# ShardianLabs/EphemeralNet

Measured on AMD Instinct MI355X. Metric: GiB/s ChaCha20-Poly1305 seal+open (device-resident) at 1/2/4/8 MI355X, higher is better.
Workload: dtype u32; 1 GPU; C2: 65536 x 4096 B records, per-record (key, nonce), AEAD seal+open, device-resident; records_per_gpu=65536, record_bytes=4096, lanes_per_record=2, parallelism=records split over 1 GPU(s), no collective

## Files before the change

### ephemeralnet_amd/build.py

```python
from __future__ import annotations

import hashlib
import json
import os
import platform
import re
import subprocess
import sys
import time
from concurrent.futures import ThreadPoolExecutor

PKG = os.path.dirname(os.path.abspath(__file__))
ROOT = os.path.dirname(PKG)
CSRC = os.path.join(PKG, "csrc")
LIB = os.path.join(PKG, "libenet_crypto.so")
OBJ = os.path.join(PKG, "build")
LIB_TOOLS = os.path.join(PKG, "libenet_crypto_tools.so")
OBJ_TOOLS = os.path.join(PKG, "build_tools")
SOURCES = ["records.hip", "segments.hip", "stream.hip", "sha.hip", "pow.hip", "duplex.hip", "duplex_split.hip",
           "chunk_frames.hip", "announce_frames.hip", "control_frames.hip",
           "shamir.hip", "shamir_host.cpp", "handshake.hip",
           "capi.cpp", "long_records.cpp", "chunk_hybrid.cpp", "staging.cpp", "scalar_api.cpp", "batch_records.cpp",
           "batch_staged.cpp", "pipeline.cpp", "host_engine.cpp",
           "frame_queue.cpp", "queue_core.cpp", "host_batch.cpp", "host_topo.cpp"]
HEADERS = ["enet_device.hpp", "enet_internal.hpp", "long_route.hpp", "record_route.hpp", "long_records.hpp", "records_body.hpp",
           "stream_common.hpp", "stream_map.hpp", "duplex_common.hpp", "pow_common.hpp", "host_engine.hpp", "scalar.hpp", "staging.hpp", "api_common.hpp", "host_batch.hpp", "host_topo.hpp", "gf256.hpp",
           "queue_knobs.hpp", "wire_host.hpp", "queue_slots.hpp", "queue_core.hpp"]
HIPCC = os.environ.get("HIPCC", "/opt/rocm/bin/hipcc")
CFLAGS = ["--offload-arch=gfx950", "-O3", "-std=c++20", "-fPIC",
          "-fvisibility=hidden", "-Wall", "-Wno-unused-function",
          "-I" + os.path.join(ROOT, "include")]
LDFLAGS = ["--offload-arch=gfx950", "-fPIC", "-shared"]


DEVICE_HEADERS = ["enet_device.hpp", "enet_internal.hpp", "long_route.hpp", "record_route.hpp", "records_body.hpp", "stream_common.hpp",
                  "stream_map.hpp", "duplex_common.hpp", "pow_common.hpp", "chacha_lockstep_asm.hpp", "gf256.hpp"]


def _headers(src: str = "") -> list[str]:
    if src.endswith(".hip"):
        return [os.path.join(CSRC, f) for f in DEVICE_HEADERS if os.path.exists(os.path.join(CSRC, f))]
    deps = [os.path.join(CSRC, f) for f in HEADERS + ["chacha_lockstep_asm.hpp"]]
    for dp, _, fs in os.walk(os.path.join(ROOT, "include")):
        deps += [os.path.join(dp, f) for f in fs]
    return [d for d in deps if os.path.exists(d)]


def _obj(src: str, obj_dir: str = OBJ) -> str:
    return os.path.join(obj_dir, os.path.splitext(src)[0] + ".o")


def _reads_tools_macro(src: str) -> bool:
    todo, seen = [src], set()
    while todo:
        f = todo.pop()
        if f in seen:
            continue
        seen.add(f)
        try:
            with open(os.path.join(CSRC, f)) as fh:
                text = fh.read()
        except OSError:
            continue
        if "ENET_TOOLS_BUILD" in text:
            return True
        todo += re.findall(r'^\s*#\s*include\s*"([^"]+)"', text, re.M)
    return False


# ... 91 lines not shown
```

### ephemeralnet_amd/csrc/chacha_lockstep_asm.hpp

```cpp
#pragma once

#define ENET_LS_C0 \
    "v_add_u32_e32 %0, %0, %4\n" \
    "v_add_u32_e32 %1, %1, %5\n" \
    "v_add_u32_e32 %2, %2, %6\n" \
    "v_add_u32_e32 %3, %3, %7\n" \
    "v_add_u32_e32 %16, %16, %20\n" \
    "v_add_u32_e32 %17, %17, %21\n" \
    "v_add_u32_e32 %18, %18, %22\n" \
    "v_add_u32_e32 %19, %19, %23\n" \
    "v_xor_b32_e32 %12, %12, %0\n" \
    "v_xor_b32_e32 %13, %13, %1\n" \
    "v_xor_b32_e32 %14, %14, %2\n" \
    "v_xor_b32_e32 %15, %15, %3\n" \
    "v_xor_b32_e32 %28, %28, %16\n" \
    "v_xor_b32_e32 %29, %29, %17\n" \
    "v_xor_b32_e32 %30, %30, %18\n" \
    "v_xor_b32_e32 %31, %31, %19\n" \
    "v_alignbit_b32 %12, %12, %12, 16\n" \
    "v_alignbit_b32 %13, %13, %13, 16\n" \
    "v_alignbit_b32 %14, %14, %14, 16\n" \
    "v_alignbit_b32 %15, %15, %15, 16\n" \
    "v_alignbit_b32 %28, %28, %28, 16\n" \
    "v_alignbit_b32 %29, %29, %29, 16\n" \
// ... 370 lines not shown
    "v_alignbit_b32 %22, %22, %22, 25\n" \
    "v_alignbit_b32 %23, %23, %23, 25\n" \
    "v_alignbit_b32 %20, %20, %20, 25\n" \
    "s_barrier\n"

#define ENET_LS_D3_NB \
    "v_add_u32_e32 %10, %10, %15\n" \
    "v_add_u32_e32 %11, %11, %12\n" \
    "v_add_u32_e32 %8, %8, %13\n" \
    "v_add_u32_e32 %9, %9, %14\n" \
    "v_add_u32_e32 %26, %26, %31\n" \
    "v_add_u32_e32 %27, %27, %28\n" \
    "v_add_u32_e32 %24, %24, %29\n" \
    "v_add_u32_e32 %25, %25, %30\n" \
    "v_xor_b32_e32 %5, %5, %10\n" \
    "v_xor_b32_e32 %6, %6, %11\n" \
    "v_xor_b32_e32 %7, %7, %8\n" \
    "v_xor_b32_e32 %4, %4, %9\n" \
    "v_xor_b32_e32 %21, %21, %26\n" \
    "v_xor_b32_e32 %22, %22, %27\n" \
    "v_xor_b32_e32 %23, %23, %24\n" \
    "v_xor_b32_e32 %20, %20, %25\n" \
    "v_alignbit_b32 %5, %5, %5, 25\n" \
    "v_alignbit_b32 %6, %6, %6, 25\n" \
    "v_alignbit_b32 %7, %7, %7, 25\n" \
    "v_alignbit_b32 %4, %4, %4, 25\n" \
    "v_alignbit_b32 %21, %21, %21, 25\n" \
    "v_alignbit_b32 %22, %22, %22, 25\n" \
    "v_alignbit_b32 %23, %23, %23, 25\n" \
    "v_alignbit_b32 %20, %20, %20, 25\n"

#define ENET_LS_X32(x)                                                                    \
    : "+v"(x[0]), "+v"(x[1]), "+v"(x[2]), "+v"(x[3]), "+v"(x[4]), "+v"(x[5]), "+v"(x[6]), "+v"(x[7]), "+v"(x[8]), "+v"(x[9]), "+v"(x[10]), "+v"(x[11]), "+v"(x[12]), "+v"(x[13]), "+v"(x[14]), "+v"(x[15]), "+v"(x[16]), "+v"(x[17]), "+v"(x[18]), "+v"(x[19]), "+v"(x[20]), "+v"(x[21]), "+v"(x[22]), "+v"(x[23]), "+v"(x[24]), "+v"(x[25]), "+v"(x[26]), "+v"(x[27]), "+v"(x[28]), "+v"(x[29]), "+v"(x[30]), "+v"(x[31])
```

### ephemeralnet_amd/csrc/enet_device.hpp

```cpp
#pragma once

#include <hip/hip_runtime.h>
#include <stdint.h>

#include <type_traits>
#include <utility>

#include "chacha_lockstep_asm.hpp"

namespace enet {

constexpr uint32_t kSigma0 = 0x61707865u, kSigma1 = 0x3320646eu, kSigma2 = 0x79622d32u,
                   kSigma3 = 0x6b206574u;

__device__ __forceinline__ uint32_t rotl(uint32_t v, int s) { return __builtin_rotateleft32(v, s); }

#define ENET_QR(a, b, c, d)                  \
    do {                                     \
        a += b; d ^= a; d = rotl(d, 16);     \
        c += d; b ^= c; b = rotl(b, 12);     \
        a += b; d ^= a; d = rotl(d, 8);      \
        c += d; b ^= c; b = rotl(b, 7);      \
    } while (0)

struct ChachaRecord {
    uint32_t k[8];
    uint32_t n[3];
    uint32_t pre[12];
};

__device__ __forceinline__ void chacha_record_init(ChachaRecord& R, const uint32_t k[8],
                                                   const uint32_t n[3]) {
#pragma unroll
    for (int i = 0; i < 8; ++i) R.k[i] = k[i];
#pragma unroll
    for (int i = 0; i < 3; ++i) R.n[i] = n[i];
    uint32_t a1 = kSigma1, b1 = k[1], c1 = k[5], d1 = n[0];
    uint32_t a2 = kSigma2, b2 = k[2], c2 = k[6], d2 = n[1];
    uint32_t a3 = kSigma3, b3 = k[3], c3 = k[7], d3 = n[2];
    ENET_QR(a1, b1, c1, d1);
    ENET_QR(a2, b2, c2, d2);
    ENET_QR(a3, b3, c3, d3);
    R.pre[0] = a1; R.pre[1] = b1; R.pre[2] = c1; R.pre[3] = d1;
    R.pre[4] = a2; R.pre[5] = b2; R.pre[6] = c2; R.pre[7] = d2;
    R.pre[8] = a3; R.pre[9] = b3; R.pre[10] = c3; R.pre[11] = d3;
}

__device__ __forceinline__ void chacha_block(const ChachaRecord& R, uint32_t counter,
                                             uint32_t x[16]) {
    uint32_t x0 = kSigma0, x4 = R.k[0], x8 = R.k[4], x12 = counter;
    ENET_QR(x0, x4, x8, x12);
    uint32_t x1 = R.pre[0], x5 = R.pre[1], x9 = R.pre[2], x13 = R.pre[3];
    uint32_t x2 = R.pre[4], x6 = R.pre[5], x10 = R.pre[6], x14 = R.pre[7];
    uint32_t x3 = R.pre[8], x7 = R.pre[9], x11 = R.pre[10], x15 = R.pre[11];
    ENET_QR(x0, x5, x10, x15);
    ENET_QR(x1, x6, x11, x12);
    ENET_QR(x2, x7, x8, x13);
    ENET_QR(x3, x4, x9, x14);
#pragma unroll
    for (int i = 1; i < 10; ++i) {
        ENET_QR(x0, x4, x8, x12);
        ENET_QR(x1, x5, x9, x13);
        ENET_QR(x2, x6, x10, x14);
        ENET_QR(x3, x7, x11, x15);
        ENET_QR(x0, x5, x10, x15);
        ENET_QR(x1, x6, x11, x12);
        ENET_QR(x2, x7, x8, x13);
        ENET_QR(x3, x4, x9, x14);
    }
    x[0] = x0 + kSigma0; x[1] = x1 + kSigma1; x[2] = x2 + kSigma2; x[3] = x3 + kSigma3;
    x[4] = x4 + R.k[0]; x[5] = x5 + R.k[1]; x[6] = x6 + R.k[2]; x[7] = x7 + R.k[3];
    x[8] = x8 + R.k[4]; x[9] = x9 + R.k[5]; x[10] = x10 + R.k[6]; x[11] = x11 + R.k[7];
    x[12] = x12 + counter; x[13] = x13 + R.n[0]; x[14] = x14 + R.n[1]; x[15] = x15 + R.n[2];
}

__device__ __forceinline__ void chacha_block2(const ChachaRecord& R, uint32_t ca, uint32_t cb,
                                              uint32_t xa[16], uint32_t xb[16]) {
    uint32_t a0 = kSigma0, a4 = R.k[0], a8 = R.k[4], a12 = ca;
// ... 78 lines not shown
    auto after = [&](auto k) {
        asm volatile("" ::: "memory");
        sh(std::integral_constant<int, BASE + decltype(k)::value>{});
        asm volatile("" ::: "memory");
    };
    constexpr bool b0 = BAR == 1, b1 = BAR == 1 || BAR == 2, b2 = BAR == 1, b3 = BAR != 0;
#define ENET_LS_STEP(NAME, B)                               \
    do {                                                    \
        if constexpr (B) asm volatile(NAME ENET_LS_X32(x)); \
        else asm volatile(NAME##_NB ENET_LS_X32(x));        \
    } while (0)
    if constexpr (DIAG) {
        ENET_LS_STEP(ENET_LS_D0, b0);
        after(std::integral_constant<int, 0>{});
        ENET_LS_STEP(ENET_LS_D1, b1);
        after(std::integral_constant<int, 1>{});
        ENET_LS_STEP(ENET_LS_D2, b2);
        after(std::integral_constant<int, 2>{});
        ENET_LS_STEP(ENET_LS_D3, b3);
        after(std::integral_constant<int, 3>{});
    } else {
        ENET_LS_STEP(ENET_LS_C0, b0);
        after(std::integral_constant<int, 0>{});
        ENET_LS_STEP(ENET_LS_C1, b1);
        after(std::integral_constant<int, 1>{});
        ENET_LS_STEP(ENET_LS_C2, b2);
        after(std::integral_constant<int, 2>{});
        ENET_LS_STEP(ENET_LS_C3, b3);
        after(std::integral_constant<int, 3>{});
    }
#undef ENET_LS_STEP
}

__device__ __forceinline__ void chacha_block2_lockstep(const ChachaRecord& R, uint32_t ca, uint32_t cb,
                                                       uint32_t xa[16], uint32_t xb[16]) {
    uint32_t a0 = kSigma0, a4 = R.k[0], a8 = R.k[4], a12 = ca;
    uint32_t b0 = kSigma0, b4 = R.k[0], b8 = R.k[4], b12 = cb;
    ENET_QR(a0, a4, a8, a12);
    ENET_QR(b0, b4, b8, b12);
    uint32_t x[32];
    x[0] = a0; x[4] = a4; x[8] = a8; x[12] = a12;
    x[16] = b0; x[20] = b4; x[24] = b8; x[28] = b12;
#pragma unroll
    for (int c = 1; c < 4; ++c) {
#pragma unroll
        for (int r = 0; r < 4; ++r) {
            x[c + 4 * r] = R.pre[4 * (c - 1) + r];
            x[16 + c + 4 * r] = R.pre[4 * (c - 1) + r];
        }
    }
    chacha_half_lockstep2<true>(x);
#pragma unroll
    for (int i = 1; i < 10; ++i) {
        chacha_half_lockstep2<false>(x);
        chacha_half_lockstep2<true>(x);
    }
    const uint32_t ff[16] = {kSigma0, kSigma1, kSigma2, kSigma3, R.k[0], R.k[1], R.k[2], R.k[3],
                             R.k[4], R.k[5], R.k[6], R.k[7], 0u, R.n[0], R.n[1], R.n[2]};
#pragma unroll
    for (int i = 0; i < 16; ++i) {
        xa[i] = x[i] + (i == 12 ? ca : ff[i]);
        xb[i] = x[16 + i] + (i == 12 ? cb : ff[i]);
    }
}

constexpr uint32_t M26 = 0x3ffffffu;
// ... 50 lines not shown
    uint32_t h0 = hin[0], h1 = hin[1], h2 = hin[2], h3 = hin[3], h4 = hin[4], c;
#pragma unroll
    for (int pass = 0; pass < 2; ++pass) {
        c = h0 >> 26; h0 &= M26; h1 += c;
        c = h1 >> 26; h1 &= M26; h2 += c;
        c = h2 >> 26; h2 &= M26; h3 += c;
        c = h3 >> 26; h3 &= M26; h4 += c;
        c = h4 >> 26; h4 &= M26; h0 += c * 5u;
    }
    c = h0 >> 26; h0 &= M26; h1 += c;
    uint32_t g0 = h0 + 5u; c = g0 >> 26; g0 &= M26;
    uint32_t g1 = h1 + c; c = g1 >> 26; g1 &= M26;
    uint32_t g2 = h2 + c; c = g2 >> 26; g2 &= M26;
    uint32_t g3 = h3 + c; c = g3 >> 26; g3 &= M26;
    uint32_t g4 = h4 + c - (1u << 26);
    const uint32_t use_g = (g4 >> 31) - 1u;
    h0 = (h0 & ~use_g) | (g0 & use_g);
    h1 = (h1 & ~use_g) | (g1 & use_g);
    h2 = (h2 & ~use_g) | (g2 & use_g);
    h3 = (h3 & ~use_g) | (g3 & use_g);
    h4 = (h4 & ~use_g) | (g4 & use_g);
    uint64_t f;
    f = (uint64_t)(h0 | (h1 << 26)) + s[0]; tag[0] = (uint32_t)f;
    f = (uint64_t)((h1 >> 6) | (h2 << 20)) + s[1] + (f >> 32); tag[1] = (uint32_t)f;
    f = (uint64_t)((h2 >> 12) | (h3 << 14)) + s[2] + (f >> 32); tag[2] = (uint32_t)f;
    f = (uint64_t)((h3 >> 18) | (h4 << 8)) + s[3] + (f >> 32); tag[3] = (uint32_t)f;
}

__device__ __forceinline__ void pclamp(uint32_t r[5], uint32_t w0, uint32_t w1, uint32_t w2,
                                       uint32_t w3) {
    plimbs(r, w0 & 0x0fffffffu, w1 & 0x0ffffffcu, w2 & 0x0ffffffcu, w3 & 0x0ffffffcu);
}

struct PolyR32 {
    uint32_t r0, r1, r2, r3, s1, s2, s3;
};

__device__ __forceinline__ PolyR32 polyr32_make(uint32_t w0, uint32_t w1, uint32_t w2, uint32_t w3) {
    PolyR32 R;
    R.r0 = w0 & 0x0fffffffu;
    R.r1 = w1 & 0x0ffffffcu;
    R.r2 = w2 & 0x0ffffffcu;
    R.r3 = w3 & 0x0ffffffcu;
    R.s1 = R.r1 + (R.r1 >> 2);
    R.s2 = R.r2 + (R.r2 >> 2);
    R.s3 = R.r3 + (R.r3 >> 2);
    return R;
}

__device__ __forceinline__ void poly32_block(uint32_t h[5], const PolyR32& R, uint32_t m0,
                                             uint32_t m1, uint32_t m2, uint32_t m3,
                                             uint32_t hibit) {
    unsigned cy;
    const uint32_t a0 = __builtin_addc(h[0], m0, 0u, &cy);
    const uint32_t a1 = __builtin_addc(h[1], m1, cy, &cy);
    const uint32_t a2 = __builtin_addc(h[2], m2, cy, &cy);
    const uint32_t a3 = __builtin_addc(h[3], m3, cy, &cy);
    const uint32_t a4 = h[4] + hibit + cy;
    const uint64_t d0 = (uint64_t)a0 * R.r0 + (uint64_t)a1 * R.s3 + (uint64_t)a2 * R.s2 +
                        (uint64_t)a3 * R.s1;
    const uint64_t e1 = (uint64_t)a0 * R.r1 + (uint64_t)a1 * R.r0 + (uint64_t)a2 * R.s3 +
                        (uint64_t)a3 * R.s2 + (uint64_t)a4 * R.s1;
    const uint64_t e2 = (uint64_t)a0 * R.r2 + (uint64_t)a1 * R.r1 + (uint64_t)a2 * R.r0 +
                        (uint64_t)a3 * R.s3 + (uint64_t)a4 * R.s2;
    const uint64_t e3 = (uint64_t)a0 * R.r3 + (uint64_t)a1 * R.r2 + (uint64_t)a2 * R.r1 +
                        (uint64_t)a3 * R.r0 + (uint64_t)a4 * R.s3;
    const uint32_t x0 = (uint32_t)d0;
    const uint32_t x1 = __builtin_addc((uint32_t)e1, (uint32_t)(d0 >> 32), 0u, &cy);
    const uint32_t c1 = (uint32_t)(e1 >> 32) + cy;
    const uint32_t x2 = __builtin_addc((uint32_t)e2, c1, 0u, &cy);
    const uint32_t c2 = (uint32_t)(e2 >> 32) + cy;
    const uint32_t x3 = __builtin_addc((uint32_t)e3, c2, 0u, &cy);
    const uint32_t c3 = (uint32_t)(e3 >> 32) + cy;
    const uint32_t t4 = a4 * R.r0 + c3;
    const uint32_t f = (t4 >> 2) * 5u;
    h[0] = __builtin_addc(x0, f, 0u, &cy);
    h[1] = __builtin_addc(x1, 0u, cy, &cy);
    h[2] = __builtin_addc(x2, 0u, cy, &cy);
    h[3] = __builtin_addc(x3, 0u, cy, &cy);
    h[4] = (t4 & 3u) + cy;
}

__device__ __forceinline__ void h32_to_limbs(const uint32_t h[5], uint32_t l[5]) {
    l[0] = h[0] & M26;
    l[1] = __builtin_amdgcn_alignbit(h[1], h[0], 26) & M26;
    l[2] = __builtin_amdgcn_alignbit(h[2], h[1], 20) & M26;
    l[3] = __builtin_amdgcn_alignbit(h[3], h[2], 14) & M26;
    l[4] = (h[3] >> 8) | (h[4] << 24);
}

__device__ __forceinline__ void ppow(const uint32_t r[5], uint32_t e, uint32_t x[5]) {
#pragma unroll
    for (int i = 0; i < 5; ++i) x[i] = r[i];
    const Pmul mr = pmul_make(r);
    const int top = 31 - __builtin_clz(e);
    for (int b = top - 1; b >= 0; --b) {
        pmul(x, pmul_make(x));
        if ((e >> b) & 1u) pmul(x, mr);
    }
}

__device__ __forceinline__ uint32_t bswap32(uint32_t v) { return __builtin_bswap32(v); }
__device__ __forceinline__ uint32_t rotr(uint32_t v, int s) { return __builtin_rotateright32(v, s); }

__constant__ static const uint32_t kSha256K[64] = {
    0x428a2f98u, 0x71374491u, 0xb5c0fbcfu, 0xe9b5dba5u, 0x3956c25bu, 0x59f111f1u, 0x923f82a4u,
    0xab1c5ed5u, 0xd807aa98u, 0x12835b01u, 0x243185beu, 0x550c7dc3u, 0x72be5d74u, 0x80deb1feu,
    0x9bdc06a7u, 0xc19bf174u, 0xe49b69c1u, 0xefbe4786u, 0x0fc19dc6u, 0x240ca1ccu, 0x2de92c6fu,
    0x4a7484aau, 0x5cb0a9dcu, 0x76f988dau, 0x983e5152u, 0xa831c66du, 0xb00327c8u, 0xbf597fc7u,
    0xc6e00bf3u, 0xd5a79147u, 0x06ca6351u, 0x14292967u, 0x27b70a85u, 0x2e1b2138u, 0x4d2c6dfcu,
    0x53380d13u, 0x650a7354u, 0x766a0abbu, 0x81c2c92eu, 0x92722c85u, 0xa2bfe8a1u, 0xa81a664bu,
    0xc24b8b70u, 0xc76c51a3u, 0xd192e819u, 0xd6990624u, 0xf40e3585u, 0x106aa070u, 0x19a4c116u,
    0x1e376c08u, 0x2748774cu, 0x34b0bcb5u, 0x391c0cb3u, 0x4ed8aa4au, 0x5b9cca4fu, 0x682e6ff3u,
    0x748f82eeu, 0x78a5636fu, 0x84c87814u, 0x8cc70208u, 0x90befffau, 0xa4506cebu, 0xbef9a3f7u,
    0xc67178f2u};
// ... 210 lines not shown
```

### ephemeralnet_amd/csrc/stream.hip

```cpp
#include "record_route.hpp"
#include "stream_common.hpp"
#include "stream_map.hpp"

namespace enet {

static_assert(kMapLanes == kStreamLanes && kMapRun == kRun, "stream_map.hpp and the streaming kernel disagree");

struct StreamSched {
    int dA, dE, sA, sE;
};
__device__ constexpr StreamSched stream_sched(int v) {
    return v == 1 ? StreamSched{1, 2, 2, 2} : v == 2 ? StreamSched{1, 4, 3, 4}
         : v == 3 ? StreamSched{1, 1, 18, 3} : v == 4 ? StreamSched{1, 2, 2, 2}
         : v == 5 ? StreamSched{1, 1, 1, 1} : StreamSched{1, 3, 2, 3};
}
__device__ constexpr int stream_barf(int v) { return v == 4 ? 2 : v == 5 ? 4 : 1; }
#ifndef ENET_STREAM_ISSUE
#define ENET_STREAM_ISSUE 30
#endif
struct StreamIssue {
    int prio_old, prio_young, prio_mem, poly;
};
__device__ constexpr StreamIssue stream_issue(int v) {
    int k = -1, poly = 0;
    if (v >= 20 && v < 28) k = v - 20;
    else if (v >= 30 && v <= 32) poly = v - 29;
    if (k < 0) return StreamIssue{0, 0, 3, poly};
    const int c = k & 3;
    return StreamIssue{c == 0 ? 0 : c == 3 ? 2 : 1, c == 1 ? 0 : c == 3 ? 2 : 1, (k & 4) ? 2 : 3, poly};
}
__device__ constexpr int stream_stores_after(StreamSched sc) {
    int n = 0;
    for (int s = 0; s < 16; ++s) n += (sc.sA + sc.sE * s >= sc.dA + 15 * sc.dE) ? 1 : 0;
    return n;
}

__device__ __forceinline__ void stream_where(const RecParams& p, int logp, uint32_t wave, uint32_t lane,
                                             uint64_t t_entry) {
    if (lane != 0 || !p.tag_out) return;
    const uint32_t hw = __builtin_amdgcn_s_getreg(4 | (31 << 11));
    uint32_t* d = reinterpret_cast<uint32_t*>(p.tag_out + 16ull * ((blockIdx.x * kStreamLanes) >> logp) + 16u * wave);
    d[0] = (uint32_t)t_entry; d[1] = (uint32_t)(t_entry >> 32); d[2] = hw; d[3] = wave;
}

template <int LOGP, int MODE, int SCHED = 0>
__global__ __launch_bounds__(kStreamWG) void stream_kernel(RecParams p) {
    constexpr StreamSched SC = stream_sched(SCHED);
    constexpr int BARF = stream_barf(SCHED);
    constexpr int kPos = kStreamSteps / BARF;
    constexpr uint32_t P = 1u << LOGP;
    constexpr bool kPoly = (MODE != MODE_XOR);
    constexpr StreamIssue ISS = stream_issue(SCHED < 20 ? ENET_STREAM_ISSUE : SCHED);
// ... 108 lines not shown
            constexpr int kStoresAfter = stream_stores_after(SC);
            uint64_t tw0 = 0;
            if (__builtin_expect(dbg & 2048, 0)) tw0 = __builtin_amdgcn_s_memtime();
            if (__builtin_expect(prev, 1)) asm volatile("s_waitcnt vmcnt(%0)" :: "n"(kStoresAfter) : "memory");
            else asm volatile("s_waitcnt vmcnt(0)" ::: "memory");
            if (__builtin_expect(dbg & 2048, 0)) wait_cyc += __builtin_amdgcn_s_memtime() - tw0;
        }
        if (__builtin_expect(dbg & 2048, 0) && lane == 0 && p.tag_out)
            reinterpret_cast<uint64_t*>(p.tag_out)[blockIdx.x * 4u + m] = wait_cyc;
        stream_barrier();
        if (S > 0 && mem) {
            uint8_t* olast = obase + (size_t)kRun * (S - 1);
#pragma unroll
            for (int s = 0; s < 16; ++s) store(olast, s, ldsread(s));
        }
        asm volatile("s_waitcnt vmcnt(0)" ::: "memory");
        stream_barrier();
        if (__builtin_expect(dbg & 32768, 0)) stream_where(p, LOGP, wave, lane, t_entry);
        return;
    }

    const uint32_t msw = slab_sw(lane);
    if (__builtin_expect(stamp, 0)) stamps[2] = __builtin_amdgcn_s_memtime();

    uint32_t kw[8], nw[3];
    {
        const uint32_t* kp = reinterpret_cast<const uint32_t*>(p.keys + (size_t)p.key_stride * rec);
#pragma unroll
        for (int i = 0; i < 8; ++i) kw[i] = kp[i];
        const uint32_t* np = reinterpret_cast<const uint32_t*>(p.nonces + 12ull * rec);
#pragma unroll
        for (int i = 0; i < 3; ++i) nw[i] = np[i];
    }
    ChachaRecord R;
    chacha_record_init(R, kw, nw);
    uint32_t ctr = 1u;
    if (MODE == MODE_XOR)
        ctr = p.counters ? p.counters[(size_t)rec * (p.counter_stride ? p.counter_stride : 1u)] : 0u;
    ctr += j * B;

    uint64_t clk0 = 0, rt0 = 0;
    if (dbg & 256) {
        clk0 = __builtin_amdgcn_s_memtime();
        rt0 = __builtin_amdgcn_s_memrealtime();
    }

    uint32_t h[5] = {0, 0, 0, 0, 0};
    PolyR32 PR{};
    uint32_t pad[4] = {0, 0, 0, 0};
    uint32_t na = 0, aad_len = 0;
    const uint32_t q = threadIdx.x & (kRecs - 1u);
    if (kPoly) {
        uint64_t aoff = 0;
        if (p.aad) {
            aoff = p.aad_off[rec];
            aad_len = (uint32_t)(p.aad_off[rec + 1] - aoff);
        }
        na = (aad_len + 15) >> 4;
        if (j == 0) {
            uint32_t otk[16];
            chacha_block(R, 0u, otk);
            PR = polyr32_make(otk[0], otk[1], otk[2], otk[3]);
            pad[0] = otk[4]; pad[1] = otk[5]; pad[2] = otk[6]; pad[3] = otk[7];
            if (kXch) s_r[q] = make_uint4(PR.r0, PR.r1, PR.r2, PR.r3);
            for (uint32_t s = 0; s < na; ++s) {
                const uint8_t* ap = p.aad + aoff + 16ull * s;
                const uint32_t cnt = min(16u, aad_len - 16u * s);
                uint32_t w[4];
// ... 12 lines not shown

    const uint32_t ff[16] = {kSigma0, kSigma1, kSigma2, kSigma3, R.k[0], R.k[1], R.k[2], R.k[3],
                             R.k[4], R.k[5], R.k[6], R.k[7], 0u, R.n[0], R.n[1], R.n[2]};
    if constexpr (ISS.prio_old == ISS.prio_young) {
        if constexpr (ISS.prio_old != 0) __builtin_amdgcn_s_setprio(ISS.prio_old);
    } else if (wave >= 4u) {
        if constexpr (ISS.prio_young != 0) __builtin_amdgcn_s_setprio(ISS.prio_young);
    } else {
        if constexpr (ISS.prio_old != 0) __builtin_amdgcn_s_setprio(ISS.prio_old);
    }
    asm volatile("s_waitcnt lgkmcnt(0)" ::: "memory");
    stream_barrier();
    if (__builtin_expect(stamp, 0)) stamps[3] = __builtin_amdgcn_s_memtime();
    if (kXch && j != 0) {
        const uint4 r = s_r[q];
        PR = polyr32_make(r.x, r.y, r.z, r.w);
    }
    for (uint32_t st = 0;;) {
        uint8_t* myrun = s_in + threadIdx.x * kRun;
        uint32_t w[32];
        if (__builtin_expect(dbg & 32, 0)) {
#pragma unroll
            for (int k = 0; k < 32; ++k) w[k] = k * lane + st;
        } else {
#pragma unroll
            for (int k = 0; k < 8; ++k) {
                const uint4 v = *reinterpret_cast<const uint4*>(myrun + 16u * (k ^ msw));
                w[4 * k] = v.x; w[4 * k + 1] = v.y; w[4 * k + 2] = v.z; w[4 * k + 3] = v.w;
            }
        }
        const uint32_t c0 = ctr + 2u * st;
        uint32_t x[32];
        {
            uint32_t a0 = kSigma0, a4 = R.k[0], a8 = R.k[4], a12 = c0;
            uint32_t b0 = kSigma0, b4 = R.k[0], b8 = R.k[4], b12 = c0 + 1u;
            ENET_QR(a0, a4, a8, a12);
            ENET_QR(b0, b4, b8, b12);
            x[0] = a0; x[4] = a4; x[8] = a8; x[12] = a12;
            x[16] = b0; x[20] = b4; x[24] = b8; x[28] = b12;
#pragma unroll
            for (int c = 1; c < 4; ++c) {
#pragma unroll
                for (int r = 0; r < 4; ++r) {
                    x[c + 4 * r] = R.pre[4 * (c - 1) + r];
                    x[16 + c + 4 * r] = R.pre[4 * (c - 1) + r];
                }
            }
        }
        asm volatile("s_waitcnt lgkmcnt(0)" ::: "memory");
        if (__builtin_expect(dbg & 2, 0)) {
#pragma unroll
            for (int k = 0; k < kPos; ++k) stream_barrier();
        } else if constexpr (MODE == MODE_OPEN && ISS.poly >= 2) {
            using Hook = PolySpreadHook<ISS.poly == 2>;
            constexpr int HB = ISS.poly == 2 ? 0 : 1;
            Hook hook(h, PR, w);
            chacha_half_lockstep2<true, Hook&, HB, 0>(x, hook);
            [&]<int... DR>(std::integer_sequence<int, DR...>) {
                ((chacha_half_lockstep2<false, Hook&, HB, 8 * DR + 4>(x, hook),
                  chacha_half_lockstep2<true, Hook&, HB, 8 * DR + 8>(x, hook)), ...);
            }(std::make_integer_sequence<int, 9>{});
        } else {
            chacha_half_lockstep2<true, NoStepHook, BARF>(x);
#pragma unroll
            for (int dr = 1; dr < 10; ++dr) {
                chacha_half_lockstep2<false, NoStepHook, BARF>(x);
                chacha_half_lockstep2<true, NoStepHook, BARF>(x);
            }
        }
        if constexpr (MODE == MODE_OPEN && ISS.poly == 1) {
#pragma unroll
            for (int i = 0; i < 32; ++i) ENET_PIN(w[i]);
        }
        if (MODE == MODE_OPEN && ISS.poly < 2 && !(dbg & 4)) {
            poly_block64(h, PR, w);
            poly_block64(h, PR, w + 16);
        }
#pragma unroll
        for (int i = 0; i < 16; ++i) {
            w[i] ^= x[i] + (i == 12 ? c0 : ff[i]);
            w[16 + i] ^= x[16 + i] + (i == 12 ? c0 + 1u : ff[i]);
        }
        if (MODE == MODE_SEAL && !(dbg & 4)) {
            poly_block64(h, PR, w);
            poly_block64(h, PR, w + 16);
        }
        uint8_t* myout = s_out + threadIdx.x * kRun;
        if (__builtin_expect(dbg & 32, 0)) {
            uint32_t acc = 0;
#pragma unroll
            for (int k = 0; k < 32; ++k) acc ^= w[k];
            if (acc == 0x9e3779b9u) myout[0] = 1;
        } else {
#pragma unroll
            for (int k = 0; k < 8; ++k)
                *reinterpret_cast<uint4*>(myout + 16u * (k ^ msw)) =
                    make_uint4(w[4 * k], w[4 * k + 1], w[4 * k + 2], w[4 * k + 3]);
        }
        if (kPoly) {
#pragma unroll
            for (int i = 0; i < 5; ++i) ENET_PIN(h[i]);
        }
        if (++st == S) break;
        asm volatile("s_waitcnt lgkmcnt(0)" ::: "memory");
        stream_barrier();
        if (__builtin_expect(stamp, 0)) stamps[3 + st] = __builtin_amdgcn_s_memtime();
    }
    uint32_t l[5] = {0, 0, 0, 0, 0};
    if (kPoly) {
        const uint32_t nct = L >> 4;
        const uint32_t N = na + nct + 1;
        if (j == P - 1) poly32_block(h, PR, aad_len, 0u, L, 0u, 1u);
        h32_to_limbs(h, l);
        if (j != P - 1) {
            const uint32_t e = N - 1 - (na + 4 * (j + 1) * B - 1);
            uint32_t r26[5], xx[5];
            plimbs(r26, PR.r0, PR.r1, PR.r2, PR.r3);
            ppow(r26, e, xx);
// ... 107 lines not shown
```

Before: 940.9 GiB/s.

## Precompute nonce-invariant first-diagonal ChaCha work and route Poly1305 through r32 helper

Extends the per-record ChaCha state with precomputed values (sigma+key sum and partial first-diagonal-round terms that depend only on key and nonce), and adds specialised inline-asm first-diagonal steps that consume these constants instead of recomputing them each block. The column-round setup also skips the first add and no longer copies pre[] into x before the rounds. Poly1305 is moved into a shared header with an optional MAD-chained variant, which is off by default, so the stream kernel calls the 32-bit block function directly. This trims a few VALU ops per 64-byte block at the cost of a few more live registers for the precomputed terms.

```diff
diff --git a/ephemeralnet_amd/build.py b/ephemeralnet_amd/build.py
--- a/ephemeralnet_amd/build.py
+++ b/ephemeralnet_amd/build.py
@@ -24,7 +24,7 @@
            "batch_staged.cpp", "pipeline.cpp", "host_engine.cpp",
            "frame_queue.cpp", "queue_core.cpp", "host_batch.cpp", "host_topo.cpp"]
 HEADERS = ["enet_device.hpp", "enet_internal.hpp", "long_route.hpp", "record_route.hpp", "long_records.hpp", "records_body.hpp",
-           "stream_common.hpp", "stream_map.hpp", "duplex_common.hpp", "pow_common.hpp", "host_engine.hpp", "scalar.hpp", "staging.hpp", "api_common.hpp", "host_batch.hpp", "host_topo.hpp", "gf256.hpp",
+           "stream_common.hpp", "stream_map.hpp", "poly1305_r32.hpp", "duplex_common.hpp", "pow_common.hpp", "host_engine.hpp", "scalar.hpp", "staging.hpp", "api_common.hpp", "host_batch.hpp", "host_topo.hpp", "gf256.hpp",
            "queue_knobs.hpp", "wire_host.hpp", "queue_slots.hpp", "queue_core.hpp"]
 HIPCC = os.environ.get("HIPCC", "/opt/rocm/bin/hipcc")
 CFLAGS = ["--offload-arch=gfx950", "-O3", "-std=c++20", "-fPIC",
@@ -34,7 +34,7 @@
 
 
 DEVICE_HEADERS = ["enet_device.hpp", "enet_internal.hpp", "long_route.hpp", "record_route.hpp", "records_body.hpp", "stream_common.hpp",
-                  "stream_map.hpp", "duplex_common.hpp", "pow_common.hpp", "chacha_lockstep_asm.hpp", "gf256.hpp"]
+                  "stream_map.hpp", "poly1305_r32.hpp", "duplex_common.hpp", "pow_common.hpp", "chacha_lockstep_asm.hpp", "gf256.hpp"]
 
 
 def _headers(src: str = "") -> list[str]:
diff --git a/ephemeralnet_amd/csrc/chacha_lockstep_asm.hpp b/ephemeralnet_amd/csrc/chacha_lockstep_asm.hpp
--- a/ephemeralnet_amd/csrc/chacha_lockstep_asm.hpp
+++ b/ephemeralnet_amd/csrc/chacha_lockstep_asm.hpp
@@ -426,3 +426,158 @@
 
 #define ENET_LS_X32(x)                                                                    \
     : "+v"(x[0]), "+v"(x[1]), "+v"(x[2]), "+v"(x[3]), "+v"(x[4]), "+v"(x[5]), "+v"(x[6]), "+v"(x[7]), "+v"(x[8]), "+v"(x[9]), "+v"(x[10]), "+v"(x[11]), "+v"(x[12]), "+v"(x[13]), "+v"(x[14]), "+v"(x[15]), "+v"(x[16]), "+v"(x[17]), "+v"(x[18]), "+v"(x[19]), "+v"(x[20]), "+v"(x[21]), "+v"(x[22]), "+v"(x[23]), "+v"(x[24]), "+v"(x[25]), "+v"(x[26]), "+v"(x[27]), "+v"(x[28]), "+v"(x[29]), "+v"(x[30]), "+v"(x[31])
+
+#define ENET_LS_D0F \
+    "v_add_u32_e32 %0, %0, %14\n" \
+    "v_add_u32_e32 %1, %15, %2\n" \
+    "v_add_u32_e32 %7, %7, %14\n" \
+    "v_add_u32_e32 %8, %15, %9\n" \
+    "v_xor_b32_e32 %6, %16, %0\n" \
+    "v_xor_b32_e32 %4, %4, %17\n" \
+    "v_xor_b32_e32 %5, %18, %1\n" \
+    "v_xor_b32_e32 %13, %16, %7\n" \
+    "v_xor_b32_e32 %11, %11, %17\n" \
+    "v_xor_b32_e32 %12, %18, %8\n" \
+    "v_alignbit_b32 %6, %6, %6, 16\n" \
+    "v_alignbit_b32 %4, %4, %4, 16\n" \
+    "v_alignbit_b32 %5, %5, %5, 16\n" \
+    "v_alignbit_b32 %13, %13, %13, 16\n" \
+    "v_alignbit_b32 %11, %11, %11, 16\n" \
+    "v_alignbit_b32 %12, %12, %12, 16\n" \
+    "s_barrier\n"
+
+#define ENET_LS_D0F_NB \
+    "v_add_u32_e32 %0, %0, %14\n" \
+    "v_add_u32_e32 %1, %15, %2\n" \
+    "v_add_u32_e32 %7, %7, %14\n" \
+    "v_add_u32_e32 %8, %15, %9\n" \
+    "v_xor_b32_e32 %6, %16, %0\n" \
+    "v_xor_b32_e32 %4, %4, %17\n" \
+    "v_xor_b32_e32 %5, %18, %1\n" \
+    "v_xor_b32_e32 %13, %16, %7\n" \
+    "v_xor_b32_e32 %11, %11, %17\n" \
+    "v_xor_b32_e32 %12, %18, %8\n" \
+    "v_alignbit_b32 %6, %6, %6, 16\n" \
+    "v_alignbit_b32 %4, %4, %4, 16\n" \
+    "v_alignbit_b32 %5, %5, %5, 16\n" \
+    "v_alignbit_b32 %13, %13, %13, 16\n" \
+    "v_alignbit_b32 %11, %11, %11, 16\n" \
+    "v_alignbit_b32 %12, %12, %12, 16\n"
+
+#define ENET_LS_D0F_OPS(x, R) \
+    : "+v"(x[0]), "=&v"(x[3]), "+v"(x[4]), "+v"(x[8]), "+v"(x[12]), "=&v"(x[14]), "=&v"(x[15]), "+v"(x[16]), "=&v"(x[19]), "+v"(x[20]), "+v"(x[24]), "+v"(x[28]), "=&v"(x[30]), "=&v"(x[31]) \
+    : "v"((R).pre[1]), "v"((R).pre[8]), "v"((R).pre[11]), "v"((R).d1[0]), "v"((R).pre[7])
+
+#define ENET_LS_D1F \
+    "v_add_u32_e32 %8, %26, %12\n" \
+    "v_add_u32_e32 %9, %27, %10\n" \
+    "v_add_u32_e32 %6, %6, %28\n" \
+    "v_add_u32_e32 %7, %29, %11\n" \
+    "v_add_u32_e32 %21, %26, %25\n" \
+    "v_add_u32_e32 %22, %27, %23\n" \
+    "v_add_u32_e32 %19, %19, %28\n" \
+    "v_add_u32_e32 %20, %29, %24\n" \
+    "v_xor_b32_e32 %3, %30, %8\n" \
+    "v_xor_b32_e32 %4, %31, %9\n" \
+    "v_xor_b32_e32 %5, %32, %6\n" \
+    "v_xor_b32_e32 %2, %2, %7\n" \
+    "v_xor_b32_e32 %16, %30, %21\n" \
+    "v_xor_b32_e32 %17, %31, %22\n" \
+    "v_xor_b32_e32 %18, %32, %19\n" \
+    "v_xor_b32_e32 %15, %15, %20\n" \
+    "v_alignbit_b32 %3, %3, %3, 20\n" \
+    "v_alignbit_b32 %4, %4, %4, 20\n" \
+    "v_alignbit_b32 %5, %5, %5, 20\n" \
+    "v_alignbit_b32 %2, %2, %2, 20\n" \
+    "v_alignbit_b32 %16, %16, %16, 20\n" \
+    "v_alignbit_b32 %17, %17, %17, 20\n" \
+    "v_alignbit_b32 %18, %18, %18, 20\n" \
+    "v_alignbit_b32 %15, %15, %15, 20\n" \
+    "s_barrier\n"
+
+#define ENET_LS_D1F_NB \
+    "v_add_u32_e32 %8, %26, %12\n" \
+    "v_add_u32_e32 %9, %27, %10\n" \
+    "v_add_u32_e32 %6, %6, %28\n" \
+    "v_add_u32_e32 %7, %29, %11\n" \
+    "v_add_u32_e32 %21, %26, %25\n" \
+    "v_add_u32_e32 %22, %27, %23\n" \
+    "v_add_u32_e32 %19, %19, %28\n" \
+    "v_add_u32_e32 %20, %29, %24\n" \
+    "v_xor_b32_e32 %3, %30, %8\n" \
+    "v_xor_b32_e32 %4, %31, %9\n" \
+    "v_xor_b32_e32 %5, %32, %6\n" \
+    "v_xor_b32_e32 %2, %2, %7\n" \
+    "v_xor_b32_e32 %16, %30, %21\n" \
+    "v_xor_b32_e32 %17, %31, %22\n" \
+    "v_xor_b32_e32 %18, %32, %19\n" \
+    "v_xor_b32_e32 %15, %15, %20\n" \
+    "v_alignbit_b32 %3, %3, %3, 20\n" \
+    "v_alignbit_b32 %4, %4, %4, 20\n" \
+    "v_alignbit_b32 %5, %5, %5, 20\n" \
+    "v_alignbit_b32 %2, %2, %2, 20\n" \
+    "v_alignbit_b32 %16, %16, %16, 20\n" \
+    "v_alignbit_b32 %17, %17, %17, 20\n" \
+    "v_alignbit_b32 %18, %18, %18, 20\n" \
+    "v_alignbit_b32 %15, %15, %15, 20\n"
+
+#define ENET_LS_D1F_OPS(x, R) \
+    : "+v"(x[0]), "+v"(x[3]), "+v"(x[4]), "=&v"(x[5]), "=&v"(x[6]), "=&v"(x[7]), "+v"(x[8]), "=&v"(x[9]), "=&v"(x[10]), "=&v"(x[11]), "+v"(x[12]), "+v"(x[14]), "+v"(x[15]), "+v"(x[16]), "+v"(x[19]), "+v"(x[20]), "=&v"(x[21]), "=&v"(x[22]), "=&v"(x[23]), "+v"(x[24]), "=&v"(x[25]), "=&v"(x[26]), "=&v"(x[27]), "+v"(x[28]), "+v"(x[30]), "+v"(x[31]) \
+    : "v"((R).pre[6]), "v"((R).pre[10]), "v"((R).d1[2]), "v"((R).pre[2]), "v"((R).pre[1]), "v"((R).pre[5]), "v"((R).pre[9])
+
+#define ENET_LS_D2F \
+    "v_add_u32_e32 %0, %0, %5\n" \
+    "v_add_u32_e32 %1, %32, %6\n" \
+    "v_add_u32_e32 %2, %33, %7\n" \
+    "v_add_u32_e32 %3, %3, %4\n" \
+    "v_add_u32_e32 %16, %16, %21\n" \
+    "v_add_u32_e32 %17, %32, %22\n" \
+    "v_add_u32_e32 %18, %33, %23\n" \
+    "v_add_u32_e32 %19, %19, %20\n" \
+    "v_xor_b32_e32 %15, %15, %0\n" \
+    "v_xor_b32_e32 %12, %12, %1\n" \
+    "v_xor_b32_e32 %13, %34, %2\n" \
+    "v_xor_b32_e32 %14, %14, %3\n" \
+    "v_xor_b32_e32 %31, %31, %16\n" \
+    "v_xor_b32_e32 %28, %28, %17\n" \
+    "v_xor_b32_e32 %29, %34, %18\n" \
+    "v_xor_b32_e32 %30, %30, %19\n" \
+    "v_alignbit_b32 %15, %15, %15, 24\n" \
+    "v_alignbit_b32 %12, %12, %12, 24\n" \
+    "v_alignbit_b32 %13, %13, %13, 24\n" \
+    "v_alignbit_b32 %14, %14, %14, 24\n" \
+    "v_alignbit_b32 %31, %31, %31, 24\n" \
+    "v_alignbit_b32 %28, %28, %28, 24\n" \
+    "v_alignbit_b32 %29, %29, %29, 24\n" \
+    "v_alignbit_b32 %30, %30, %30, 24\n" \
+    "s_barrier\n"
+
+#define ENET_LS_D2F_NB \
+    "v_add_u32_e32 %0, %0, %5\n" \
+    "v_add_u32_e32 %1, %32, %6\n" \
+    "v_add_u32_e32 %2, %33, %7\n" \
+    "v_add_u32_e32 %3, %3, %4\n" \
+    "v_add_u32_e32 %16, %16, %21\n" \
+    "v_add_u32_e32 %17, %32, %22\n" \
+    "v_add_u32_e32 %18, %33, %23\n" \
+    "v_add_u32_e32 %19, %19, %20\n" \
+    "v_xor_b32_e32 %15, %15, %0\n" \
+    "v_xor_b32_e32 %12, %12, %1\n" \
+    "v_xor_b32_e32 %13, %34, %2\n" \
+    "v_xor_b32_e32 %14, %14, %3\n" \
+    "v_xor_b32_e32 %31, %31, %16\n" \
+    "v_xor_b32_e32 %28, %28, %17\n" \
+    "v_xor_b32_e32 %29, %34, %18\n" \
+    "v_xor_b32_e32 %30, %30, %19\n" \
+    "v_alignbit_b32 %15, %15, %15, 24\n" \
+    "v_alignbit_b32 %12, %12, %12, 24\n" \
+    "v_alignbit_b32 %13, %13, %13, 24\n" \
+    "v_alignbit_b32 %14, %14, %14, 24\n" \
+    "v_alignbit_b32 %31, %31, %31, 24\n" \
+    "v_alignbit_b32 %28, %28, %28, 24\n" \
+    "v_alignbit_b32 %29, %29, %29, 24\n" \
+    "v_alignbit_b32 %30, %30, %30, 24\n"
+
+#define ENET_LS_D2F_OPS(x, R) \
+    : "+v"(x[0]), "=&v"(x[1]), "=&v"(x[2]), "+v"(x[3]), "+v"(x[4]), "+v"(x[5]), "+v"(x[6]), "+v"(x[7]), "+v"(x[8]), "+v"(x[9]), "+v"(x[10]), "+v"(x[11]), "+v"(x[12]), "=&v"(x[13]), "+v"(x[14]), "+v"(x[15]), "+v"(x[16]), "=&v"(x[17]), "=&v"(x[18]), "+v"(x[19]), "+v"(x[20]), "+v"(x[21]), "+v"(x[22]), "+v"(x[23]), "+v"(x[24]), "+v"(x[25]), "+v"(x[26]), "+v"(x[27]), "+v"(x[28]), "=&v"(x[29]), "+v"(x[30]), "+v"(x[31]) \
+    : "v"((R).d1[0]), "v"((R).d1[1]), "v"((R).d1[2])
diff --git a/ephemeralnet_amd/csrc/enet_device.hpp b/ephemeralnet_amd/csrc/enet_device.hpp
--- a/ephemeralnet_amd/csrc/enet_device.hpp
+++ b/ephemeralnet_amd/csrc/enet_device.hpp
@@ -7,6 +7,7 @@
 #include <utility>
 
 #include "chacha_lockstep_asm.hpp"
+#include "poly1305_r32.hpp"
 
 namespace enet {
 
@@ -18,6 +19,14 @@
 #define ENET_QR(a, b, c, d)                  \
     do {                                     \
         a += b; d ^= a; d = rotl(d, 16);     \
+        c += d; b ^= c; b = rotl(b, 12);     \
+        a += b; d ^= a; d = rotl(d, 8);      \
+        c += d; b ^= c; b = rotl(b, 7);      \
+    } while (0)
+
+#define ENET_QR_ADDED(a, b, c, d)            \
+    do {                                     \
+        d ^= a; d = rotl(d, 16);             \
         c += d; b ^= c; b = rotl(b, 12);     \
         a += b; d ^= a; d = rotl(d, 8);      \
         c += d; b ^= c; b = rotl(b, 7);      \
@@ -44,6 +53,20 @@
     R.pre[0] = a1; R.pre[1] = b1; R.pre[2] = c1; R.pre[3] = d1;
     R.pre[4] = a2; R.pre[5] = b2; R.pre[6] = c2; R.pre[7] = d2;
     R.pre[8] = a3; R.pre[9] = b3; R.pre[10] = c3; R.pre[11] = d3;
+}
+
+struct ChachaStageRecord : ChachaRecord {
+    uint32_t s0k;
+    uint32_t d1[3];
+};
+
+__device__ __forceinline__ void chacha_stage_record_init(ChachaStageRecord& R, const uint32_t k[8],
+                                                         const uint32_t n[3]) {
+    chacha_record_init(R, k, n);
+    R.s0k = kSigma0 + k[0];
+    R.d1[0] = R.pre[0] + R.pre[5];
+    R.d1[1] = R.pre[4] + R.pre[9];
+    R.d1[2] = rotl(R.pre[3] ^ R.d1[1], 16);
 }
 
 __device__ __forceinline__ void chacha_block(const ChachaRecord& R, uint32_t counter,
@@ -188,6 +211,32 @@
 #undef ENET_LS_STEP
 }
 
+template <class SH = NoStepHook, int BAR = 1, int BASE = 0>
+__device__ __forceinline__ void chacha_first_diag_lockstep2(uint32_t x[32], const ChachaStageRecord& R,
+                                                            SH&& sh = SH{}) {
+    auto after = [&](auto k) {
+        asm volatile("" ::: "memory");
+        sh(std::integral_constant<int, BASE + decltype(k)::value>{});
+        asm volatile("" ::: "memory");
+    };
+    constexpr bool b0 = BAR == 1, b1 = BAR == 1 || BAR == 2, b2 = BAR == 1, b3 = BAR != 0;
+#define ENET_LS_STEP_F(NAME, B)                                   \
+    do {                                                          \
+        if constexpr (B) asm volatile(NAME NAME##_OPS(x, R));     \
+        else asm volatile(NAME##_NB NAME##_OPS(x, R));            \
+    } while (0)
+    ENET_LS_STEP_F(ENET_LS_D0F, b0);
+    after(std::integral_constant<int, 0>{});
+    ENET_LS_STEP_F(ENET_LS_D1F, b1);
+    after(std::integral_constant<int, 1>{});
+    ENET_LS_STEP_F(ENET_LS_D2F, b2);
+    after(std::integral_constant<int, 2>{});
+#undef ENET_LS_STEP_F
+    if constexpr (b3) asm volatile(ENET_LS_D3 ENET_LS_X32(x));
+    else asm volatile(ENET_LS_D3_NB ENET_LS_X32(x));
+    after(std::integral_constant<int, 3>{});
+}
+
 __device__ __forceinline__ void chacha_block2_lockstep(const ChachaRecord& R, uint32_t ca, uint32_t cb,
                                                        uint32_t xa[16], uint32_t xb[16]) {
     uint32_t a0 = kSigma0, a4 = R.k[0], a8 = R.k[4], a12 = ca;
@@ -304,55 +353,6 @@
     plimbs(r, w0 & 0x0fffffffu, w1 & 0x0ffffffcu, w2 & 0x0ffffffcu, w3 & 0x0ffffffcu);
 }
 
-struct PolyR32 {
-    uint32_t r0, r1, r2, r3, s1, s2, s3;
-};
-
-__device__ __forceinline__ PolyR32 polyr32_make(uint32_t w0, uint32_t w1, uint32_t w2, uint32_t w3) {
-    PolyR32 R;
-    R.r0 = w0 & 0x0fffffffu;
-    R.r1 = w1 & 0x0ffffffcu;
-    R.r2 = w2 & 0x0ffffffcu;
-    R.r3 = w3 & 0x0ffffffcu;
-    R.s1 = R.r1 + (R.r1 >> 2);
-    R.s2 = R.r2 + (R.r2 >> 2);
-    R.s3 = R.r3 + (R.r3 >> 2);
-    return R;
-}
-
-__device__ __forceinline__ void poly32_block(uint32_t h[5], const PolyR32& R, uint32_t m0,
-                                             uint32_t m1, uint32_t m2, uint32_t m3,
-                                             uint32_t hibit) {
-    unsigned cy;
-    const uint32_t a0 = __builtin_addc(h[0], m0, 0u, &cy);
-    const uint32_t a1 = __builtin_addc(h[1], m1, cy, &cy);
-    const uint32_t a2 = __builtin_addc(h[2], m2, cy, &cy);
-    const uint32_t a3 = __builtin_addc(h[3], m3, cy, &cy);
-    const uint32_t a4 = h[4] + hibit + cy;
-    const uint64_t d0 = (uint64_t)a0 * R.r0 + (uint64_t)a1 * R.s3 + (uint64_t)a2 * R.s2 +
-                        (uint64_t)a3 * R.s1;
-    const uint64_t e1 = (uint64_t)a0 * R.r1 + (uint64_t)a1 * R.r0 + (uint64_t)a2 * R.s3 +
-                        (uint64_t)a3 * R.s2 + (uint64_t)a4 * R.s1;
-    const uint64_t e2 = (uint64_t)a0 * R.r2 + (uint64_t)a1 * R.r1 + (uint64_t)a2 * R.r0 +
-                        (uint64_t)a3 * R.s3 + (uint64_t)a4 * R.s2;
-    const uint64_t e3 = (uint64_t)a0 * R.r3 + (uint64_t)a1 * R.r2 + (uint64_t)a2 * R.r1 +
-                        (uint64_t)a3 * R.r0 + (uint64_t)a4 * R.s3;
-    const uint32_t x0 = (uint32_t)d0;
-    const uint32_t x1 = __builtin_addc((uint32_t)e1, (uint32_t)(d0 >> 32), 0u, &cy);
-    const uint32_t c1 = (uint32_t)(e1 >> 32) + cy;
-    const uint32_t x2 = __builtin_addc((uint32_t)e2, c1, 0u, &cy);
-    const uint32_t c2 = (uint32_t)(e2 >> 32) + cy;
-    const uint32_t x3 = __builtin_addc((uint32_t)e3, c2, 0u, &cy);
-    const uint32_t c3 = (uint32_t)(e3 >> 32) + cy;
-    const uint32_t t4 = a4 * R.r0 + c3;
-    const uint32_t f = (t4 >> 2) * 5u;
-    h[0] = __builtin_addc(x0, f, 0u, &cy);
-    h[1] = __builtin_addc(x1, 0u, cy, &cy);
-    h[2] = __builtin_addc(x2, 0u, cy, &cy);
-    h[3] = __builtin_addc(x3, 0u, cy, &cy);
-    h[4] = (t4 & 3u) + cy;
-}
-
 __device__ __forceinline__ void h32_to_limbs(const uint32_t h[5], uint32_t l[5]) {
     l[0] = h[0] & M26;
     l[1] = __builtin_amdgcn_alignbit(h[1], h[0], 26) & M26;
diff --git a/ephemeralnet_amd/csrc/poly1305_r32.hpp b/ephemeralnet_amd/csrc/poly1305_r32.hpp
--- /dev/null
+++ b/ephemeralnet_amd/csrc/poly1305_r32.hpp
@@ -0,0 +1,111 @@
+#pragma once
+
+#include <stdint.h>
+
+#if defined(__HIPCC__)
+#define ENET_POLY_FN __host__ __device__ __forceinline__
+#else
+#define ENET_POLY_FN inline
+#endif
+
+#if defined(__has_builtin)
+#if __has_builtin(__builtin_addc)
+#define ENET_POLY_HAS_ADDC 1
+#endif
+#endif
+
+#if defined(__HIP_DEVICE_COMPILE__)
+#define ENET_POLY_HOLD(v) asm volatile("" : "+v"(v))
+#else
+#define ENET_POLY_HOLD(v) ((void)0)
+#endif
+
+namespace enet {
+
+ENET_POLY_FN uint32_t poly_addc(uint32_t a, uint32_t b, unsigned cin, unsigned* cout) {
+#ifdef ENET_POLY_HAS_ADDC
+    return __builtin_addc(a, b, cin, cout);
+#else
+    const uint64_t s = (uint64_t)a + b + cin;
+    *cout = (unsigned)(s >> 32);
+    return (uint32_t)s;
+#endif
+}
+
+struct PolyR32 {
+    uint32_t r0, r1, r2, r3, s1, s2, s3;
+};
+
+ENET_POLY_FN PolyR32 polyr32_make(uint32_t w0, uint32_t w1, uint32_t w2, uint32_t w3) {
+    PolyR32 R;
+    R.r0 = w0 & 0x0fffffffu;
+    R.r1 = w1 & 0x0ffffffcu;
+    R.r2 = w2 & 0x0ffffffcu;
+    R.r3 = w3 & 0x0ffffffcu;
+    R.s1 = R.r1 + (R.r1 >> 2);
+    R.s2 = R.r2 + (R.r2 >> 2);
+    R.s3 = R.r3 + (R.r3 >> 2);
+    return R;
+}
+
+ENET_POLY_FN void poly32_block(uint32_t h[5], const PolyR32& R, uint32_t m0, uint32_t m1, uint32_t m2,
+                               uint32_t m3, uint32_t hibit) {
+    unsigned cy;
+    const uint32_t a0 = poly_addc(h[0], m0, 0u, &cy);
+    const uint32_t a1 = poly_addc(h[1], m1, cy, &cy);
+    const uint32_t a2 = poly_addc(h[2], m2, cy, &cy);
+    const uint32_t a3 = poly_addc(h[3], m3, cy, &cy);
+    const uint32_t a4 = h[4] + hibit + cy;
+    const uint64_t d0 = (uint64_t)a0 * R.r0 + (uint64_t)a1 * R.s3 + (uint64_t)a2 * R.s2 +
+                        (uint64_t)a3 * R.s1;
+    const uint64_t e1 = (uint64_t)a0 * R.r1 + (uint64_t)a1 * R.r0 + (uint64_t)a2 * R.s3 +
+                        (uint64_t)a3 * R.s2 + (uint64_t)a4 * R.s1;
+    const uint64_t e2 = (uint64_t)a0 * R.r2 + (uint64_t)a1 * R.r1 + (uint64_t)a2 * R.r0 +
+                        (uint64_t)a3 * R.s3 + (uint64_t)a4 * R.s2;
+    const uint64_t e3 = (uint64_t)a0 * R.r3 + (uint64_t)a1 * R.r2 + (uint64_t)a2 * R.r1 +
+                        (uint64_t)a3 * R.r0 + (uint64_t)a4 * R.s3;
+    const uint32_t x0 = (uint32_t)d0;
+    const uint32_t x1 = poly_addc((uint32_t)e1, (uint32_t)(d0 >> 32), 0u, &cy);
+    const uint32_t c1 = (uint32_t)(e1 >> 32) + cy;
+    const uint32_t x2 = poly_addc((uint32_t)e2, c1, 0u, &cy);
+    const uint32_t c2 = (uint32_t)(e2 >> 32) + cy;
+    const uint32_t x3 = poly_addc((uint32_t)e3, c2, 0u, &cy);
+    const uint32_t c3 = (uint32_t)(e3 >> 32) + cy;
+    const uint32_t t4 = a4 * R.r0 + c3;
+    const uint32_t f = (t4 >> 2) * 5u;
+    h[0] = poly_addc(x0, f, 0u, &cy);
+    h[1] = poly_addc(x1, 0u, cy, &cy);
+    h[2] = poly_addc(x2, 0u, cy, &cy);
+    h[3] = poly_addc(x3, 0u, cy, &cy);
+    h[4] = (t4 & 3u) + cy;
+}
+
+ENET_POLY_FN void poly32_block_mad(uint32_t h[5], const PolyR32& R, uint32_t m0, uint32_t m1, uint32_t m2,
+                                   uint32_t m3, uint32_t hibit) {
+    unsigned cy;
+    const uint32_t a0 = poly_addc(h[0], m0, 0u, &cy);
+    const uint32_t a1 = poly_addc(h[1], m1, cy, &cy);
+    const uint32_t a2 = poly_addc(h[2], m2, cy, &cy);
+    const uint32_t a3 = poly_addc(h[3], m3, cy, &cy);
+    const uint32_t a4 = h[4] + hibit + cy;
+    const uint64_t d0 = (uint64_t)a0 * R.r0 + (uint64_t)a1 * R.s3 + (uint64_t)a2 * R.s2 +
+                        (uint64_t)a3 * R.s1;
+    uint64_t e1 = (uint64_t)a0 * R.r1 + (d0 >> 32);
+    ENET_POLY_HOLD(e1);
+    e1 += (uint64_t)a1 * R.r0 + (uint64_t)a2 * R.s3 + (uint64_t)a3 * R.s2 + (uint64_t)a4 * R.s1;
+    uint64_t e2 = (uint64_t)a0 * R.r2 + (e1 >> 32);
+    ENET_POLY_HOLD(e2);
+    e2 += (uint64_t)a1 * R.r1 + (uint64_t)a2 * R.r0 + (uint64_t)a3 * R.s3 + (uint64_t)a4 * R.s2;
+    uint64_t e3 = (uint64_t)a0 * R.r3 + (e2 >> 32);
+    ENET_POLY_HOLD(e3);
+    e3 += (uint64_t)a1 * R.r2 + (uint64_t)a2 * R.r1 + (uint64_t)a3 * R.r0 + (uint64_t)a4 * R.s3;
+    const uint32_t t4 = a4 * R.r0 + (uint32_t)(e3 >> 32);
+    const uint32_t f = (t4 >> 2) * 5u;
+    h[0] = poly_addc((uint32_t)d0, f, 0u, &cy);
+    h[1] = poly_addc((uint32_t)e1, 0u, cy, &cy);
+    h[2] = poly_addc((uint32_t)e2, 0u, cy, &cy);
+    h[3] = poly_addc((uint32_t)e3, 0u, cy, &cy);
+    h[4] = (t4 & 3u) + cy;
+}
+
+}
diff --git a/ephemeralnet_amd/csrc/stream.hip b/ephemeralnet_amd/csrc/stream.hip
--- a/ephemeralnet_amd/csrc/stream.hip
+++ b/ephemeralnet_amd/csrc/stream.hip
@@ -18,6 +18,16 @@
 #ifndef ENET_STREAM_ISSUE
 #define ENET_STREAM_ISSUE 30
 #endif
+#ifndef ENET_STREAM_POLY_MAD
+#define ENET_STREAM_POLY_MAD 0
+#endif
+__device__ __forceinline__ void stream_poly_block64(uint32_t h[5], const PolyR32& R, const uint32_t ct[16]) {
+#pragma unroll
+    for (int u = 0; u < 4; ++u) {
+        if constexpr (ENET_STREAM_POLY_MAD) poly32_block_mad(h, R, ct[4 * u], ct[4 * u + 1], ct[4 * u + 2], ct[4 * u + 3], 1u);
+        else poly32_block(h, R, ct[4 * u], ct[4 * u + 1], ct[4 * u + 2], ct[4 * u + 3], 1u);
+    }
+}
 struct StreamIssue {
     int prio_old, prio_young, prio_mem, poly;
 };
@@ -192,8 +202,8 @@
 #pragma unroll
         for (int i = 0; i < 3; ++i) nw[i] = np[i];
     }
-    ChachaRecord R;
-    chacha_record_init(R, kw, nw);
+    ChachaStageRecord R;
+    chacha_stage_record_init(R, kw, nw);
     uint32_t ctr = 1u;
     if (MODE == MODE_XOR)
         ctr = p.counters ? p.counters[(size_t)rec * (p.counter_stride ? p.counter_stride : 1u)] : 0u;
@@ -272,36 +282,33 @@
         const uint32_t c0 = ctr + 2u * st;
         uint32_t x[32];
         {
-            uint32_t a0 = kSigma0, a4 = R.k[0], a8 = R.k[4], a12 = c0;
-            uint32_t b0 = kSigma0, b4 = R.k[0], b8 = R.k[4], b12 = c0 + 1u;
-            ENET_QR(a0, a4, a8, a12);
-            ENET_QR(b0, b4, b8, b12);
+            uint32_t a0 = R.s0k, a4 = R.k[0], a8 = R.k[4], a12 = c0;
+            uint32_t b0 = R.s0k, b4 = R.k[0], b8 = R.k[4], b12 = c0 + 1u;
+            ENET_QR_ADDED(a0, a4, a8, a12);
+            ENET_QR_ADDED(b0, b4, b8, b12);
             x[0] = a0; x[4] = a4; x[8] = a8; x[12] = a12;
             x[16] = b0; x[20] = b4; x[24] = b8; x[28] = b12;
-#pragma unroll
-            for (int c = 1; c < 4; ++c) {
-#pragma unroll
-                for (int r = 0; r < 4; ++r) {
-                    x[c + 4 * r] = R.pre[4 * (c - 1) + r];
-                    x[16 + c + 4 * r] = R.pre[4 * (c - 1) + r];
-                }
-            }
         }
         asm volatile("s_waitcnt lgkmcnt(0)" ::: "memory");
         if (__builtin_expect(dbg & 2, 0)) {
+#pragma unroll
+            for (int c = 1; c < 4; ++c) {
+#pragma unroll
+                for (int r = 0; r < 4; ++r) x[c + 4 * r] = x[16 + c + 4 * r] = R.pre[4 * (c - 1) + r];
+            }
 #pragma unroll
             for (int k = 0; k < kPos; ++k) stream_barrier();
         } else if constexpr (MODE == MODE_OPEN && ISS.poly >= 2) {
             using Hook = PolySpreadHook<ISS.poly == 2>;
             constexpr int HB = ISS.poly == 2 ? 0 : 1;
             Hook hook(h, PR, w);
-            chacha_half_lockstep2<true, Hook&, HB, 0>(x, hook);
+            chacha_first_diag_lockstep2<Hook&, HB, 0>(x, R, hook);
             [&]<int... DR>(std::integer_sequence<int, DR...>) {
                 ((chacha_half_lockstep2<false, Hook&, HB, 8 * DR + 4>(x, hook),
                   chacha_half_lockstep2<true, Hook&, HB, 8 * DR + 8>(x, hook)), ...);
             }(std::make_integer_sequence<int, 9>{});
         } else {
-            chacha_half_lockstep2<true, NoStepHook, BARF>(x);
+            chacha_first_diag_lockstep2<NoStepHook, BARF>(x, R);
 #pragma unroll
             for (int dr = 1; dr < 10; ++dr) {
                 chacha_half_lockstep2<false, NoStepHook, BARF>(x);
@@ -313,8 +320,8 @@
             for (int i = 0; i < 32; ++i) ENET_PIN(w[i]);
         }
         if (MODE == MODE_OPEN && ISS.poly < 2 && !(dbg & 4)) {
-            poly_block64(h, PR, w);
-            poly_block64(h, PR, w + 16);
+            stream_poly_block64(h, PR, w);
+            stream_poly_block64(h, PR, w + 16);
         }
 #pragma unroll
         for (int i = 0; i < 16; ++i) {
@@ -322,8 +329,8 @@
             w[16 + i] ^= x[16 + i] + (i == 12 ? c0 + 1u : ff[i]);
         }
         if (MODE == MODE_SEAL && !(dbg & 4)) {
-            poly_block64(h, PR, w);
-            poly_block64(h, PR, w + 16);
+            stream_poly_block64(h, PR, w);
+            stream_poly_block64(h, PR, w + 16);
         }
         uint8_t* myout = s_out + threadIdx.x * kRun;
         if (__builtin_expect(dbg & 32, 0)) {
```

Result: no change. 945.1 GiB/s (median of 6 runs) (+0.5%).
